# EPFL-IMOS/simple-SFOD

Measured on AMD Instinct MI355X. Metric: teacher+student train images/s on 1024x2048 synthetic, higher is better.
Workload: dtype bf16x3

## Files before the change

include/sfod_hip.h:

```cpp
#ifndef SFOD_HIP_H
#define SFOD_HIP_H
#include <stdint.h>
#ifdef __cplusplus
extern "C" {
#endif

#define SFOD_F32 0
#define SFOD_BF16 1
#define SFOD_BF16X3 2
#define SFOD_F16X3 3

int sfod_version(void);
const char* sfod_last_error(void);

int sfod_preprocess(const void* const* img_ptrs, const int32_t* sizes, int B, int Hp, int Wp,
                    int Cpad, const float* mean3, const float* std3, void* out, int dt,
                    void* stream);

int sfod_hflip_u8(const void* src, void* dst, int C, int H, int W, void* stream);

int sfod_resize_bilinear_u8(const void* src, void* dst, int C, int H, int W, int h, int w,
                            const int32_t* hbounds, const int32_t* hcoef, int ksize_h,
                            const int32_t* vbounds, const int32_t* vcoef, int ksize_v, int flip,
                            void* stream);
int sfod_resize_bilinear_u8_opt(const void* src, void* dst, int C, int H, int W, int y0, int x0, int ch, int cw,
                                int h, int w, const int32_t* hbounds, const int32_t* hcoef, int ksize_h,
                                const int32_t* vbounds, const int32_t* vcoef, int ksize_v, int flip_mode,
                                void* stream);

int sfod_conv_fwd(const void* x, const void* w, const float* bias, void* y, int B, int H, int W,
                  int Cin, int Cout, int ksize, int ldy, int act, float* stats, int dt, int out_dt,
                  void* stream);
int sfod_conv_fwd_ws(const void* x, const void* w, const uint32_t* w_absmax, const float* bias, void* y, int B, int H,
                     int W, int Cin, int Cout, int ksize, int ldy, int act, float* stats, int dt, int out_dt,
                     void* stream);
int64_t sfod_conv_fwd_scratch_bytes(int B, int H, int W, int Cin, int Cout, int ksize, int dt, int out_dt, int with_stats);
int sfod_conv_fwd_scratch(const void* x, const void* w, const uint32_t* w_absmax, const float* bias, void* y, int B, int H,
                          int W, int Cin, int Cout, int ksize, int ldy, int act, float* stats, int dt, int out_dt,
                          void* scratch, int64_t scratch_bytes, void* stream);
int sfod_conv_stats_blocks(int B, int H, int W, int Cin, int Cout, int ksize, int dt);
int sfod_set_conv_algo(int algo);
int sfod_conv_dgrad_bnred_blocks(int B, int H, int W, int Cin, int Cout, int dt);
int sfod_conv_dgrad_bnred(const void* x, const void* w, void* dz, int B, int H, int W, int Cin, int Cout, int dt,
                          const float* y, const float* mean, const float* invstd, const float* gamma,
                          const float* beta, float* red_ws, void* stream);
int sfod_conv_fwd_bnin_supported(int B, int H, int W, int Cin, int Cout, int dt);
int sfod_conv_fwd_bnin(const float* x_pre, const float* in_mean, const float* in_invstd, const float* in_gamma,
                       const float* in_beta, const void* w, const float* bias, float* y, int B, int H, int W, int Cin,
                       int Cout, int ldy, int act, float* stats, int dt, void* stream);
int sfod_set_gemm_tile(int tile);
int sfod_set_conv3x3_variant(int variant);
int sfod_last_conv_kernel(char* buf, int n);
int sfod_set_deterministic(int on);
int sfod_get_deterministic(void);
int sfod_set_conv3x3_m16(int on);
int sfod_set_wgrad3x3_pipe(int on);
int sfod_conv_fwd_algo(int B, int H, int W, int Cin, int Cout, int ksize, int dt);

int sfod_conv_first_supported(int B, int H, int W, int Cin, int Cout, int dt, int ldy);
int sfod_conv_first_fused(const void* x, const void* w, const float* bias, const float* scale,
                          const float* shift, void* y, float* stats, int B, int H, int W, int ldy,
                          int act, int dt, void* stream);
int sfod_conv_first_fused_ws(const void* x, const void* w, const uint32_t* w_absmax, const float* bias,
                             const float* scale, const float* shift, void* y, float* stats, int B, int H, int W,
                             int ldy, int act, int dt, void* stream);

int64_t sfod_conv_wgrad_ws_bytes(int B, int H, int W, int Cin, int Cout, int ksize, int lddy, int dt);
int sfod_conv_wgrad(const void* x, const void* dy, float* dw, int B, int H, int W, int Cin,
                    int Cout, int ksize, int lddy, int dt, void* ws, int64_t ws_bytes, void* stream);
int sfod_conv_wgrad_oihw_supported(int B, int H, int W, int Cin, int Cout, int ksize, int lddy, int dt);
int sfod_conv_wgrad_oihw(const void* x, const void* dy, float* dw_oihw, int B, int H, int W, int Cin,
                         int Cout, int ksize, int lddy, int dt, int accumulate, void* ws,
                         int64_t ws_bytes, void* stream);

int sfod_pack_conv_weight(const float* w_oihw, void* w_packed, int Cout, int Cin, int ksize,
                          int CinPad, int rot180, int dt, void* stream);
int sfod_pack_conv_weight_ws(const float* w_oihw, void* w_packed, uint32_t* absmax, int Cout, int Cin, int ksize,
                             int CinPad, int rot180, int dt, void* stream);
int sfod_pack_conv_weights_blocks(int Cout, int Cin, int ksize, int innerPad, int rot180);
int sfod_pack_conv_weights_multi(const int64_t* desc, int n, int total_blocks, int dt, void* stream);
int sfod_pack_conv_weights_multi_ws(const int64_t* desc, int n, int total_blocks, int dt, uint32_t* absmax ,
                                    void* stream);
int sfod_unpack_conv_wgrad(const float* dw_packed, float* dw_oihw, int Cout, int Cin, int ksize,
                           int CinPad, int accumulate, void* stream);
int sfod_pack_fc_weight(const float* w, void* out, int N, int K, int chw_c, int transpose, int dt,
                        void* stream);
int sfod_unpack_fc_wgrad(const float* dw_packed, float* dw, int N, int K, int chw_c,
                         int accumulate, void* stream);
int sfod_pack_fc_weight_ld(const float* w, void* out, int N, int K, int chw_c, int transpose, int ld,
                           int dt, void* stream);
int sfod_pack_fc_weight_ld_ws(const float* w, void* out, uint32_t* absmax, int N, int K, int chw_c, int transpose,
                              int ld, int dt, void* stream);
int sfod_unpack_fc_wgrad_ld(const float* dw_packed, float* dw, int N, int K, int chw_c, int ld,
                            int accumulate, void* stream);
int sfod_bias_grad(const void* dy, float* db, int M, int N, int ld, int accumulate, int dt,
                   void* stream);

int sfod_bn_finalize(const float* stats, int nblocks, int M, int C,
                     float* mean, float* invstd, float* running_mean, float* running_var,
                     float momentum, float eps, int update_running, int64_t* num_batches_tracked,
                     float* ws, void* stream);
int sfod_set_bn_finalize_fused(int on);
int sfod_bn_finalize_ws_floats(int C);
int sfod_bn_relu_pool_fwd(const void* y, const float* mean, const float* invstd,
                          const float* gamma, const float* beta, void* z, int B, int H, int W,
                          int C, int pool, int dt, int out_dt, void* stream);
int sfod_bn_relu_pool_fwd2(const void* y, const float* mean, const float* invstd,
                           const float* gamma, const float* beta, void* z, void* z2, int B, int H, int W,
                           int C, int pool, int dt, int out_dt, void* stream);
int sfod_bn_add_relu_fwd(const void* y, const float* mean, const float* invstd, const float* gamma,
                         const float* beta, const void* residual, void* z, void* z_pairs, void* z_pairs2, int64_t rows,
                         int C, int dt, int pairs_dt, void* stream);
int sfod_bn_relu_pool_bwd(const void* dz, const void* y, const float* mean, const float* invstd,
                          const float* gamma, const float* beta, void* dy, float* dgamma,
                          float* dbeta, float* dgamma_acc, float* dbeta_acc, float* ws, int B, int H,
                          int W, int C, int pool, int dt, int out_dt, int reduced_blocks, void* stream);
#define SFOD_BN_BWD_SCRATCH_ROWS 32
int sfod_bn_bwd_ws_floats(int M, int C);
int sfod_add_act(const void* a, const void* b, void* out, void* out_pairs, void* out_pairs2, int64_t n, int act, int dt,
                 int pairs_dt, void* stream);
int sfod_subsample2(const void* src, void* dst, int B, int H, int W, int C, int backward, int dt,
                    void* stream);
int sfod_stem7x7_supported(int B, int H, int W, int Cp, int dt);
int sfod_stem7x7(const float* x, const void* w_packed, const uint32_t* w_absmax, const float* bias, float* y, int B, int H,
                 int W, int Cp, int act, int dt, void* stream);
int sfod_im2col_stem(const void* x, void* out, int B, int H, int W, int Cp, int Kpad, int dt, int out_dt,
                     void* stream);
int sfod_maxpool3s2(const void* x, void* y, int B, int H, int W, int C, int dt, void* stream);
int sfod_act_bwd(void* dy, const void* y, int64_t n, int act, int dt, void* stream);
int sfod_add_inplace(void* a, const void* b, int64_t n, int dt, void* stream);
int sfod_add_act_bwd(void* a, const void* b, const void* y, int64_t n, int dt, void* stream);
int sfod_mul_mask(void* a, const uint8_t* mask, int64_t n, float scale, int dt, void* stream);

int sfod_rpn_decode(const float* rpn_out, int ld, const float* cell_anchors, int A, int B, int Hf,
                    int Wf, int stride, const int32_t* image_sizes, float* props, float* scores,
                    int32_t* flags, void* stream);
int sfod_rpn_decode_opt(const float* rpn_out, int ld, const float* cell_anchors, int A, int B, int Hf,
                        int Wf, int stride, const int32_t* image_sizes, float* props, float* scores,
                        int32_t* flags, float wx, float wy, float ww, float wh, void* stream);
int64_t sfod_sort_ws_bytes(int B, int n);
int sfod_segmented_sort_desc(const float* keys, int B, int n, float* out_keys, int32_t* out_idx,
                             void* ws, int64_t ws_bytes, void* stream);
int sfod_rpn_gather_topk(const float* props, const float* sorted_scores, const int32_t* sorted_idx,
                         int B, int NA, int k, float* cand_boxes, float* cand_scores,
                         uint8_t* cand_valid, void* stream);
// ... 125 lines not shown
```

simple-sfod_amd/csrc/elementwise.hip:

```cpp
#include "conv_internal.h"
#include <type_traits>
#include <atomic>
#include <stdlib.h>

template <typename T> struct VecT;
template <> struct VecT<float> {
  static constexpr int N = 4;
  typedef float4 raw;
};
template <> struct VecT<bf16_t> {
  static constexpr int N = 8;
  typedef uint4 raw;
};

template <> struct VecT<split_t> {
  static constexpr int N = 8;
  typedef uint4 raw;
};
template <> struct VecT<splith_t> {
  static constexpr int N = 8;
  typedef uint4 raw;
};

template <typename T> __device__ __forceinline__ void load_vec(const T* p, float* out);
// ... 1676 lines not shown
                                 int transpose, int ld, const unsigned* __restrict__ amax) {
  const float ws = amax != nullptr ? wscale_from_absmax(*amax) : 1.0f;
  const int rows = transpose ? K : N;
  const int64_t total = (int64_t)rows * ld;
  const int PP = chw_c > 0 ? K / chw_c : 1;
  for (int64_t t = (int64_t)blockIdx.x * blockDim.x + threadIdx.x; t < total;
       t += (int64_t)gridDim.x * blockDim.x) {
    const int inner = (int)(t % ld);
    const int row = (int)(t / ld);
    const int n = transpose ? inner : row;
    const int kp = transpose ? row : inner;
    float v = 0.f;
    if (n < N && kp < K) {
      int k = kp;
      if (chw_c > 0) { const int p = kp / chw_c, c = kp % chw_c; k = c * PP + p; }
      v = w[(int64_t)n * K + k];
    }
    put_elem<T>(out, t, v * ws);
  }
}

template <typename T>
__global__ void __launch_bounds__(256)
k_pack_fc_chw(const float* __restrict__ w, T* __restrict__ out, int N, int C, int PP, int ld,
              const unsigned* __restrict__ amax) {
  const float ws = amax != nullptr ? wscale_from_absmax(*amax) : 1.0f;
  extern __shared__ float tile[];
  const int n = blockIdx.y, c0 = blockIdx.x * 64;
  const int cw = min(64, C - c0);
  const float* src = w + (int64_t)n * C * PP + (int64_t)c0 * PP;
  for (int i = threadIdx.x; i < cw * PP; i += 256) tile[i] = src[i];
  __syncthreads();
  T* dst = out + (int64_t)n * ld;
  for (int j = threadIdx.x; j < PP * 64; j += 256) {
    const int p = j >> 6, cl = j & 63;
    if (cl < cw) put_elem<T>(dst, (int64_t)p * C + c0 + cl, tile[cl * PP + p] * ws);
  }
}

template <typename T>
__global__ void __launch_bounds__(256)
k_pack_fc_chw_t(const float* __restrict__ w, T* __restrict__ out, int N, int C, int PP, int ld,
                const unsigned* __restrict__ amax) {
  const float ws = amax != nullptr ? wscale_from_absmax(*amax) : 1.0f;
  extern __shared__ float tile[];
  const int n0 = blockIdx.y * 64, c0 = blockIdx.x * 4;
  const int nw = min(64, N - n0), cw = min(4, C - c0);
  const int run = cw * PP, pitch = 4 * PP + 1;
  for (int i = threadIdx.x; i < nw * run; i += 256) {
    const int nl = i / run, r = i - nl * run;
    tile[nl * pitch + r] = w[(int64_t)(n0 + nl) * C * PP + (int64_t)c0 * PP + r];
  }
  __syncthreads();
  for (int j = threadIdx.x; j < run * 64; j += 256) {
    const int r = j >> 6, nl = j & 63;
    if (nl < nw) {
      const int cl = r / PP, p = r - cl * PP;
      put_elem<T>(out, ((int64_t)p * C + c0 + cl) * ld + n0 + nl, tile[nl * pitch + r] * ws);
    }
  }
}

extern "C" int sfod_pack_fc_weight_ld_ws(const float* w, void* out, uint32_t* absmax, int N, int K, int chw_c,
                                         int transpose, int ld, int dt, void* stream) {
  SFOD_REQUIRE_EXTENTS("pack_fc_weight_ld_ws", N, K, chw_c, ld);
  SFOD_REQUIRE(ld >= (transpose ? N : K), "pack_fc_weight: ld too small");
  SFOD_REQUIRE(!sfod_is_pairs(dt) || ld % 8 == 0, "pack_fc_weight: operand pairs need ld % 8 == 0");
  SFOD_REQUIRE(absmax == nullptr || dt == SFOD_F16X3, "pack_fc_weight: the per-tensor scale belongs to SFOD_F16X3");
  hipStream_t s = (hipStream_t)stream;
  if (absmax != nullptr) {
    const int rc = launch_weight_absmax(w, (int64_t)N * K, nullptr, 1, absmax, s);
    if (rc) return rc;
  }
  const unsigned* am = absmax;
  const unsigned* none = nullptr;
  if (chw_c > 0 && K % chw_c == 0 && K / chw_c <= 64 && (int64_t)N * K >= (1 << 20) &&
      ld == (transpose ? N : K)) {
    const int C = chw_c, PP = K / chw_c;
    if (!transpose) {
      const dim3 grid(cdiv(C, 64), N);
      const size_t lds = (size_t)64 * PP * 4;
      if (dt == SFOD_F32) hipLaunchKernelGGL(k_pack_fc_chw<float>, grid, dim3(256), lds, s, w, (float*)out, N, C, PP, ld, none);
      else if (dt == SFOD_BF16X3) hipLaunchKernelGGL(k_pack_fc_chw<split_t>, grid, dim3(256), lds, s, w, (split_t*)out, N, C, PP, ld, none);
      else if (dt == SFOD_F16X3) hipLaunchKernelGGL(k_pack_fc_chw<splith_t>, grid, dim3(256), lds, s, w, (splith_t*)out, N, C, PP, ld, am);
      else hipLaunchKernelGGL(k_pack_fc_chw<bf16_t>, grid, dim3(256), lds, s, w, (bf16_t*)out, N, C, PP, ld, none);
    } else {
      const dim3 grid(cdiv(C, 4), cdiv(N, 64));
      const size_t lds = (size_t)64 * (4 * PP + 1) * 4;
      if (dt == SFOD_F32) hipLaunchKernelGGL(k_pack_fc_chw_t<float>, grid, dim3(256), lds, s, w, (float*)out, N, C, PP, ld, none);
      else if (dt == SFOD_BF16X3) hipLaunchKernelGGL(k_pack_fc_chw_t<split_t>, grid, dim3(256), lds, s, w, (split_t*)out, N, C, PP, ld, none);
      else if (dt == SFOD_F16X3) hipLaunchKernelGGL(k_pack_fc_chw_t<splith_t>, grid, dim3(256), lds, s, w, (splith_t*)out, N, C, PP, ld, am);
      else hipLaunchKernelGGL(k_pack_fc_chw_t<bf16_t>, grid, dim3(256), lds, s, w, (bf16_t*)out, N, C, PP, ld, none);
    }
    return sfod_check_launch("pack_fc_weight(chw)");
  }
  const int64_t total = (int64_t)(transpose ? K : N) * ld;
  if (dt == SFOD_BF16X3)
    hipLaunchKernelGGL(k_pack_fc_weight<split_t>, dim3(ew_grid(total)), dim3(256), 0, s, w, (split_t*)out, N, K, chw_c, transpose, ld, none);
  else if (dt == SFOD_F16X3)
    hipLaunchKernelGGL(k_pack_fc_weight<splith_t>, dim3(ew_grid(total)), dim3(256), 0, s, w, (splith_t*)out, N, K, chw_c, transpose, ld, am);
  else if (dt == SFOD_F32)
    hipLaunchKernelGGL(k_pack_fc_weight<float>, dim3(ew_grid(total)), dim3(256), 0, s, w, (float*)out, N, K, chw_c, transpose, ld, none);
  else
    hipLaunchKernelGGL(k_pack_fc_weight<bf16_t>, dim3(ew_grid(total)), dim3(256), 0, s, w, (bf16_t*)out, N, K, chw_c, transpose, ld, none);
  return sfod_check_launch("pack_fc_weight");
}

extern "C" int sfod_pack_fc_weight_ld(const float* w, void* out, int N, int K, int chw_c, int transpose,
                                      int ld, int dt, void* stream) {
  SFOD_REQUIRE_EXTENTS("pack_fc_weight_ld", N, K, chw_c, ld);
  return sfod_pack_fc_weight_ld_ws(w, out, nullptr, N, K, chw_c, transpose, ld, dt, stream);
}

extern "C" int sfod_pack_fc_weight(const float* w, void* out, int N, int K, int chw_c, int transpose,
                                   int dt, void* stream) {
  SFOD_REQUIRE_EXTENTS("pack_fc_weight", N, K, chw_c);
  return sfod_pack_fc_weight_ld(w, out, N, K, chw_c, transpose, transpose ? N : K, dt, stream);
}

__global__ void k_unpack_fc_wgrad(const float* __restrict__ dwp, float* __restrict__ dw, int N, int K,
                                  int chw_c, int ld, int accumulate) {
  const int64_t total = (int64_t)N * K;
  const int PP = chw_c > 0 ? K / chw_c : 1;
  for (int64_t t = (int64_t)blockIdx.x * blockDim.x + threadIdx.x; t < total;
       t += (int64_t)gridDim.x * blockDim.x) {
    const int k = (int)(t % K);
    const int n = (int)(t / K);
    int kp = k;
    if (chw_c > 0) { const int c = k / PP, p = k % PP; kp = p * chw_c + c; }
    const float v = dwp[(int64_t)n * ld + kp];
    dw[t] = accumulate ? dw[t] + v : v;
  }
}

__global__ void __launch_bounds__(256)
k_unpack_fc_chw(const float* __restrict__ dwp, float* __restrict__ dw, int C, int PP, int ld, int accumulate) {
  extern __shared__ float tile[];
  const int n = blockIdx.y, c0 = blockIdx.x * 64;
  const int cw = min(64, C - c0);
  const float* src = dwp + (int64_t)n * ld;
  for (int j = threadIdx.x; j < PP * 64; j += 256) {
    const int p = j >> 6, cl = j & 63;
    if (cl < cw) tile[cl * PP + p] = src[(int64_t)p * C + c0 + cl];
  }
  __syncthreads();
// ... 510 lines not shown
```

simple-sfod_amd/csrc/gemm_conv.hip:

```cpp
#include "conv_internal.h"
#include <algorithm>
#include <atomic>

typedef __attribute__((ext_vector_type(8))) __bf16 bf16x8;
typedef __attribute__((ext_vector_type(4))) short s16x4;
typedef __attribute__((ext_vector_type(8))) short s16x8;
typedef __attribute__((ext_vector_type(16))) float f32x16;
typedef __attribute__((ext_vector_type(4))) float f32x4;

#define LDS_PTR(p) ((__attribute__((address_space(3))) void*)(p))
#define GLB_PTR(p) ((const __attribute__((address_space(1))) void*)(p))

__device__ __attribute__((aligned(16))) unsigned int g_zero_page[64];

struct ConvArgs {
  int M;
  int H, W;
  int Cin;
  int Cout;
  int ks;
  int cpt_shift;
  int kchunks;
  int ldy;
  int act;
// ... 1257 lines not shown
        acc.x += v.x; acc.y += v.y; acc.z += v.z; acc.w += v.w;
      }
      *reinterpret_cast<float4*>(dw + i) = acc;
    } else {
      for (int64_t e = i; e < n && e < i + 4; ++e) {
        float acc = dw[e];
        for (int sl = 0; sl < nslab; ++sl) acc += ws[sl * stride + e];
        dw[e] = acc;
      }
    }
  }
}

struct GenWgradPlan { int wide, tiles_n, tiles_m, splits, pps; };
static GenWgradPlan gen_wgrad_plan(int M, int Cout, int Ntot, int dt) {
  GenWgradPlan g;
  const int split = (dt == SFOD_BF16X3);
  g.wide = split && Cout >= 128 && Ntot >= 256 && g_conv_algo != 3 &&
           (g_conv_algo == 4 || (int64_t)((Ntot + 255) / 256) * ((Cout + 127) / 128) >= 256);
  if (g.wide) {
    constexpr int BKP = 32;
    g.tiles_n = (Ntot + 255) / 256; g.tiles_m = (Cout + 127) / 128;
    const int tiles = g.tiles_n * g.tiles_m;
    const int max_splits = std::max(1, M / (8 * BKP));
    int best = 1;
    double best_eff = 0.0;
    for (int sp = 1; sp <= std::min(max_splits, 512); ++sp) {
      const int64_t wgs = (int64_t)tiles * sp;
      const double eff = (double)wgs / (double)((wgs + 255) / 256 * 256);
      if (eff > best_eff + 1e-9) { best_eff = eff; best = sp; }
      if (eff >= 0.85 && wgs >= 512) { best = sp; break; }
      if (wgs >= 4096) break;
    }
    int pps = (M + best - 1) / best;
    pps = (pps + BKP - 1) / BKP * BKP;
    g.pps = pps;
    g.splits = (M + pps - 1) / pps;
    return g;
  }
  const int BKP = (dt == SFOD_F32) ? 32 : 64;
  const int TILE = split ? 64 : 128;
  g.tiles_n = (Ntot + TILE - 1) / TILE; g.tiles_m = (Cout + TILE - 1) / TILE;
  int splits = (1024 + g.tiles_n * g.tiles_m - 1) / (g.tiles_n * g.tiles_m);
  const int max_splits = (M + BKP - 1) / BKP;
  if (splits > max_splits) splits = max_splits;
  if (splits < 1) splits = 1;
  int pps = (M + splits - 1) / splits;
  pps = (pps + BKP - 1) / BKP * BKP;
  g.pps = pps;
  g.splits = (M + pps - 1) / pps;
  return g;
}

extern "C" int64_t sfod_conv_wgrad_ws_bytes(int B, int H, int W, int Cin, int Cout, int ksize, int lddy, int dt) {
  if (!(conv_shape_fits(B, H, W, Cin, Cout, ksize) && sfod_ints_ok({lddy}))) return 0;
  int nb = 0;
  if (dt != SFOD_F32) {
    const W3Plan p = w3_plan_chunked(B, H, W, Cin, Cout, ksize, lddy, dt, nb);
    if (nb > 0) return p.ws_bytes;
  }
  if (!sfod_deterministic() || (int64_t)B * H * W == 0) return 0;
  const int Ntot = ksize * ksize * Cin;
  const GenWgradPlan g = gen_wgrad_plan(B * H * W, Cout, Ntot, dt);
  return g.splits > 1 ? (int64_t)g.splits * Cout * Ntot * 4 : 0;
}

extern "C" int sfod_conv_wgrad_oihw_supported(int B, int H, int W, int Cin, int Cout, int ksize, int lddy, int dt) {
  if (!(conv_shape_fits(B, H, W, Cin, Cout, ksize) && sfod_ints_ok({lddy}))) return 0;
  int nb;
  w3_plan_chunked(B, H, W, Cin, Cout, ksize, lddy, dt, nb);
  return nb > 0 ? 1 : 0;
}

extern "C" int sfod_conv_wgrad_oihw(const void* x, const void* dy, float* dw_oihw, int B, int H, int W, int Cin,
                                    int Cout, int ksize, int lddy, int dt, int accumulate, void* ws,
                                    int64_t ws_bytes, void* stream) {
  sfod_note_conv_kernel(nullptr);
  SFOD_REQUIRE(conv_shape_fits(B, H, W, Cin, Cout, ksize) && sfod_ints_ok({lddy}) && sfod_i64s_ok({ws_bytes}),
               "conv_wgrad_oihw: negative or oversized extent");
  SFOD_REQUIRE(x != nullptr && dy != nullptr && dw_oihw != nullptr, "conv_wgrad_oihw: null operand");
  SFOD_REQUIRE(lddy >= Cout, "conv_wgrad_oihw: lddy < Cout");
  int nb;
  w3_plan_chunked(B, H, W, Cin, Cout, ksize, lddy, dt, nb);
  SFOD_REQUIRE(nb > 0, "wgrad_oihw: shape not served by the halo-patch kernel (query sfod_conv_wgrad_oihw_supported)");
  return w3_launch_chunked(x, dy, dw_oihw, ws, ws_bytes, B, H, W, Cin, Cout, lddy, dt, accumulate ? 2 : 1, nb,
                           (hipStream_t)stream);
}

extern "C" int sfod_conv_wgrad(const void* x, const void* dy, float* dw, int B, int H, int W, int Cin,
                               int Cout, int ksize, int lddy, int dt, void* ws, int64_t ws_bytes,
                               void* stream) {
  sfod_note_conv_kernel(nullptr);
  SFOD_REQUIRE(conv_shape_fits(B, H, W, Cin, Cout, ksize) && sfod_ints_ok({lddy}) && sfod_i64s_ok({ws_bytes}),
               "conv_wgrad: negative or oversized extent");
  SFOD_REQUIRE(x != nullptr && dy != nullptr && dw != nullptr, "conv_wgrad: null operand");
  SFOD_REQUIRE(lddy >= Cout, "conv_wgrad: lddy < Cout");
  SFOD_REQUIRE(ksize == 1 || ksize == 3, "wgrad: ksize must be 1 or 3");
  SFOD_REQUIRE(dt == SFOD_F32 || dt == SFOD_BF16 || dt == SFOD_BF16X3, "wgrad: unknown dt");
  const int E = (dt == SFOD_F32) ? 4 : 8;
  SFOD_REQUIRE(Cin % E == 0 && lddy % E == 0, "wgrad: Cin / lddy must be multiples of the 16-byte chunk (bf16x3: of 8)");
  if ((int64_t)B * H * W == 0) return 0;
  const int split = (dt == SFOD_BF16X3);
  SFOD_REQUIRE(!split || Cout % 8 == 0, "wgrad: bf16x3 needs Cout % 8 == 0");
  {
    int nb;
    w3_plan_chunked(B, H, W, Cin, Cout, ksize, lddy, dt, nb);
    if (nb > 0) return w3_launch_chunked(x, dy, dw, ws, ws_bytes, B, H, W, Cin, Cout, lddy, dt, 0, nb, (hipStream_t)stream);
  }
  hipStream_t s = (hipStream_t)stream;
  float* dw_out = dw;
  WgradArgs a;
  a.M = B * H * W; a.H = H; a.W = W; a.Cin = Cin; a.Cout = Cout; a.ks = ksize; a.lddy = lddy;
  const int cpt = Cin / E;
  a.cpt_shift = 0;
  if (ksize == 3) {
    a.cpt_shift = ilog2_exact(cpt);
    SFOD_REQUIRE(a.cpt_shift >= 0, "wgrad3x3: Cin/chunk must be a power of two");
  }
  a.nchunks = ksize * ksize * cpt;
  a.Ntot = ksize * ksize * Cin;
  if (a.M == 0) return 0;
  const GenWgradPlan g = gen_wgrad_plan(a.M, Cout, a.Ntot, dt);
  a.pix_per_split = g.pps;
  a.tiles_n = g.tiles_n;
  a.tiles_m = g.tiles_m;
  a.slab_stride = 0;
  const bool slabs = sfod_deterministic() && g.splits > 1;
  if (slabs) {
    const int64_t need = (int64_t)g.splits * Cout * a.Ntot * 4;
    if (ws == nullptr || ws_bytes < need) {
      sfod_set_error("wgrad: deterministic mode needs the workspace of sfod_conv_wgrad_ws_bytes");
      return SFOD_EBADARG;
    }
    a.slab_stride = (int64_t)Cout * a.Ntot;
    dw_out = (float*)ws;
  }
  const int tiles = g.tiles_n * g.tiles_m;
  if (g.wide) {
    constexpr int LDS = 3 * 32 * (128 + 256) * 4;
    static const hipError_t attr_rc = hipFuncSetAttribute(reinterpret_cast<const void*>(k_conv_wgrad_x3w),
                                                          hipFuncAttributeMaxDynamicSharedMemorySize, LDS);
    SFOD_REQUIRE(attr_rc == hipSuccess, "wgrad: cannot raise the dynamic LDS limit");
    sfod_note_conv_kernel("k_conv_wgrad_x3w");
    hipLaunchKernelGGL(k_conv_wgrad_x3w, dim3(tiles * g.splits), dim3(512), LDS, s, (const bf16_t*)x, (const bf16_t*)dy,
                       dw_out, a);
  } else {
    dim3 grid(tiles * g.splits);
    sfod_note_conv_kernel(dt == SFOD_F32 ? "k_conv_wgrad<float,2,2,0>"
                                         : (split ? "k_conv_wgrad<bf16_t,2,2,1>" : "k_conv_wgrad<bf16_t,2,2,0>"));
    if (dt == SFOD_F32)
      hipLaunchKernelGGL((k_conv_wgrad<float, 2, 2>), grid, dim3(256), 2 * 2 * 32 * 512, s, (const float*)x,
                         (const float*)dy, dw_out, a);
    else if (split)
      hipLaunchKernelGGL((k_conv_wgrad<bf16_t, 2, 2, true>), grid, dim3(256), 2 * 2 * 64 * 256, s, (const bf16_t*)x,
                         (const bf16_t*)dy, dw_out, a);
    else
      hipLaunchKernelGGL((k_conv_wgrad<bf16_t, 2, 2>), grid, dim3(256), 2 * 2 * 64 * 256, s, (const bf16_t*)x,
                         (const bf16_t*)dy, dw_out, a);
  }
  int rc = sfod_check_launch(g.wide ? "conv_wgrad_x3w" : "conv_wgrad");
  if (rc == 0 && slabs) {
    const int64_t n = (int64_t)Cout * a.Ntot;
// ... 7 lines not shown
```

simple-sfod_amd/modeling/roi_heads.py:

```python
import math

import torch
import torch.nn as nn

from .. import native
from ..registry import ROI_BOX_HEAD_REGISTRY, ROI_HEADS_REGISTRY
from ..structures import Boxes, Instances, ShapeSpec
from .offchain import OffChain as _OffChain, heads_on as _heads_on
from .batched import BatchedDetections, BatchedGT, BatchedProposals
from .box_regression import ROI_DEFAULT_WEIGHTS, roi_box_reg_options
from .roi_pooler import roi_pooler_options


class ROIPooler(nn.Module):

    def __init__(self, output_size, scales, sampling_ratio, pooler_type, prefix="MODEL.ROI_BOX_HEAD"):
        super().__init__()
        assert len(scales) == 1
        output_size, self.sampling_ratio, self.aligned = roi_pooler_options(output_size, sampling_ratio, pooler_type, prefix)
        self.pooler_type = pooler_type
        self.options = {} if (self.sampling_ratio == 0 and self.aligned) else \
            {"sampling_ratio": self.sampling_ratio, "aligned": self.aligned}
        self.output_size = (output_size, output_size)
        self.scale = scales[0]
# ... 248 lines not shown
        pk = self.__dict__.pop("_packed", None) or {}
        pooled = native.roi_align_fwd(feat, rois, self.pooled, self.box_pooler.scale, **self.box_pooler.options)
        R = pooled.shape[0]
        x0 = pooled.view(R, PP * C)
        w1 = pk["w1"] if pk else native.pack_fc_weight(bh.fc1.weight.detach(), dt, chw_c=C)
        h1 = native.conv_fwd(x0, w1, bh.fc1.bias.detach(), bh.fc1.out_features, 1, act=1)
        w2 = pk["w2"] if pk else native.pack_fc_weight(bh.fc2.weight.detach(), dt)
        h2 = native.conv_fwd(h1, w2, bh.fc2.bias.detach(), bh.fc2.out_features, 1, act=1)
        wp = pk["wp"] if pk else torch.cat([bp.cls_score.weight.detach(), bp.bbox_pred.weight.detach()])
        bpb = pk["bpb"] if pk else torch.cat([bp.cls_score.bias.detach(), bp.bbox_pred.bias.detach()])
        wpp = pk["wpp"] if pk else native.pack_fc_weight(wp, dt)
        pred = native.conv_fwd(h2, wpp, bpb, wp.shape[0], 1, out_dtype=torch.float32, ldy=self.pred_ld)
        st = {"x0": x0, "h1": h1, "h2": h2, "pred": pred, "wp": wp, "feat_shape": tuple(feat.shape)}
        for k in ("wpt", "w2t", "w1t"):
            if k in pk:
                st[k] = pk[k]
        return st

    def _box_backward(self, st, rois, d_pred, feat_shape_nchw):
        dtype = native.grad_dtype_of(self.compute_dtype)
        dt = native.dt_of_dtype(dtype)
        bh = self.box_head
        K = self.num_classes
        NP = self.pred_cols
        d_pred_c = native.cast(d_pred, dtype)
        off = _OffChain(_heads_on(d_pred))
        dwp, dbp = off.run(lambda: (native.conv_wgrad(st["h2"], d_pred_c, NP, 1, operand=dtype).view(NP, -1),
                                    native.bias_grad(d_pred, NP)), st["h2"], d_pred_c, d_pred)
        wpt = st.get("wpt")
        if wpt is None:
            wpt = native.pack_fc_weight(st["wp"], dt, transpose=True, ld=self.pred_ld)
        dh2 = native.conv_fwd(d_pred_c, wpt, None, bh.fc2.out_features, 1)
        dfeat, (dw1, db1, dw2, db2) = self._box_head_backward(st, rois, dh2)
        off.join(dwp, dbp)
        pgrads = [dw1, db1, dw2, db2, dwp[: K + 1].contiguous(), dbp[: K + 1].contiguous(),
                  dwp[K + 1:].contiguous(), dbp[K + 1:].contiguous()]
        return dfeat, pgrads

    def _box_head_backward(self, st, rois, dh2):
        dtype = native.grad_dtype_of(self.compute_dtype)
        dt = native.dt_of_dtype(dtype)
        bh = self.box_head
        C = self.channels
        native.act_bwd_(dh2, st["h2"], 1)
        off = _OffChain(_heads_on(dh2))
        dw2, db2 = off.run(lambda: (native.conv_wgrad(st["h1"], dh2, bh.fc2.out_features, 1, operand=dtype).view(bh.fc2.out_features, -1),
                                    native.bias_grad(dh2, bh.fc2.out_features)), st["h1"], dh2)
        w2t = st.get("w2t")
        if w2t is None:
            w2t = native.pack_fc_weight(bh.fc2.weight.detach(), dt, transpose=True)
        dh1 = native.conv_fwd(dh2, w2t, None, bh.fc2.in_features, 1)
        native.act_bwd_(dh1, st["h1"], 1)
        def fc1_param_grads():
            dw1p = native.conv_wgrad(st["x0"], dh1, bh.fc1.out_features, 1, operand=dtype).view(bh.fc1.out_features, -1)
            dw1_ = native.grad_sink(bh.fc1.weight)
            if dw1_ is not None:
                native.unpack_fc_wgrad(dw1p, dw1_, chw_c=C, accumulate=True)
                dw1_ = None
            else:
                dw1_ = torch.empty_like(bh.fc1.weight)
                native.unpack_fc_wgrad(dw1p, dw1_, chw_c=C)
            return dw1_, native.bias_grad(dh1, bh.fc1.out_features)

        dw1, db1 = off.run(fc1_param_grads, st["x0"], dh1)
        w1t = st.get("w1t")
        if w1t is None:
            w1t = native.pack_fc_weight(bh.fc1.weight.detach(), dt, chw_c=C, transpose=True)
        dx0 = native.conv_fwd(dh1, w1t, None, bh.fc1.in_features, 1)
        B, H, W, _ = st["feat_shape"]
        dfeat = native.roi_align_bwd(dx0.view(-1, self.pooled * self.pooled, C), rois, (B, H, W, C), self.pooled,
                                     self.box_pooler.scale, **self.box_pooler.options)
        off.join(dw1, db1, dw2, db2)
        return dfeat.permute(0, 3, 1, 2), [dw1, db1, dw2, db2]

    @torch.no_grad()
    def label_and_sample_proposals(self, proposals, targets, branch="", keys=None):
        props = proposals
        B, P, _ = props.boxes.shape
        if self.proposal_append_gt:
            boxes, count = native.append_gt(props.boxes, props.count, targets.boxes, targets.count)
        else:
            boxes, count = props.boxes, props.count
        matched, cls = native.roi_match(boxes, count, targets.boxes, targets.classes, targets.count,
                                        self.iou_threshold, self.num_classes)
        keys = keys if keys is not None else getattr(self, "_forced_keys", None)
        if keys is None:
            keys = torch.randint(0, 2 ** 31 - 1, (B, boxes.shape[1]), dtype=torch.int32, device=boxes.device)
        sidx, scnt = native.subsample_roi(cls, keys, self.batch_size_per_image, self.positive_fraction,
                                          self.num_classes)
        rois, gt_cls, gt_box, n_valid = native.roi_build_samples(boxes, cls, matched, sidx, scnt, targets.boxes,
                                                                 targets.count)
        return {"rois": rois, "gt_cls": gt_cls, "gt_box": gt_box, "n_valid": n_valid, "count": scnt,
                "sampled_idxs": sidx, "image_sizes": props.image_sizes}

    @torch.no_grad()
    def _inference(self, feat, proposals, sizes_dev=None):
        rois = native.make_rois(proposals.boxes, proposals.count)
        st = self._box_forward(feat, rois)
        bp = self.box_predictor
        if sizes_dev is None:
            sizes_dev = native.dev_const(tuple((int(s[0]), int(s[1])) for s in proposals.image_sizes), torch.int32,
                                         feat.device)
        out = native.frcnn_inference(st["pred"], self.num_classes, proposals.boxes, proposals.count, sizes_dev,
                                     bp.test_score_thresh, bp.test_nms_thresh, bp.test_topk_per_image,
                                     self.bbox_threshold, self.nms_numel_limit, box_reg=bp._box_reg)
        return BatchedDetections(out, proposals.image_sizes), st["pred"]
# ... 60 lines not shown
```

simple-sfod_amd/native.py:

```python
import collections
import ctypes
import os
import re
import warnings

import torch

warnings.filterwarnings("ignore", message="ComplexHalf support is experimental")

_HERE = os.path.dirname(os.path.abspath(__file__))
HEADER = os.path.join(os.path.dirname(_HERE), "include", "sfod_hip.h")
SO_PATH = os.environ.get("SFOD_HIP_LIB", os.path.join(_HERE, "lib", "libsfod_hip.so"))

F32, BF16, BF16X3, F16X3 = 0, 1, 2, 3

SPLIT_DTYPE = torch.complex32
SPLITH_DTYPE = torch.uint32
PAIR_DTYPES = (SPLIT_DTYPE, SPLITH_DTYPE)

COMPUTE_MODES = {"fp32": F32, "bf16": BF16, "bf16x3": BF16X3, "f16x3": F16X3}


def mode_dt(name):
    try:
# ... 155 lines not shown
    return as_operand(t, dtype), as_operand(t, gdt)


class _Everything:
    def __contains__(self, item):
        return True


class KernelTimer:

    def __init__(self, watch=("sfod_conv_fwd", "sfod_conv_wgrad", "sfod_conv_wgrad_oihw")):
        self.watch = _Everything() if watch is None else set(watch)
        self.records = []

    def summary(self):
        torch.cuda.synchronize()
        out = {}
        for name, flops, a, b in self.records:
            d = out.setdefault(name, {"launches": 0, "ms": 0.0, "flops": 0.0})
            d["launches"] += 1
            d["ms"] += a.elapsed_time(b)
            d["flops"] += flops
        return out


_timer = None


def set_timer(timer):
    global _timer
    _timer = timer


def call(name, *args, timer_name=None, flops=0.0, tag=""):
    lib = load()
    conv = [(_p(a) if isinstance(a, torch.Tensor) else a) for a in args]
    if _timer is not None and (timer_name or name) in _timer.watch:
        a, b = torch.cuda.Event(enable_timing=True), torch.cuda.Event(enable_timing=True)
        a.record()
        rc = getattr(lib, name)(*conv, _stream())
        b.record()
        _timer.records.append(((timer_name or name) + tag, flops, a, b))
    else:
        rc = getattr(lib, name)(*conv, _stream())
    _chk(rc, name)


def query(name, *args):
    return getattr(load(), name)(*args)


def set_conv_algo(algo):
    load().sfod_set_conv_algo(int(algo))


def set_wgrad3x3_pipe(on):
    load().sfod_set_wgrad3x3_pipe(int(on))


def set_gemm_tile(tile):
    load().sfod_set_gemm_tile(int(tile))


def set_conv3x3_variant(variant):
    load().sfod_set_conv3x3_variant(int(variant))


def last_conv_kernel():
    buf = ctypes.create_string_buffer(256)
    n = load().sfod_last_conv_kernel(buf, len(buf))
    if n < 0:
        _chk(n, "sfod_last_conv_kernel")
    return buf.value.decode()


def set_deterministic(on):
    lib = load()
    prev = bool(lib.sfod_get_deterministic())
    lib.sfod_set_deterministic(int(bool(on)))
    return prev


def set_bn_finalize_fused(on):
    load().sfod_set_bn_finalize_fused(int(bool(on)))


def set_conv3x3_m16(on):
    load().sfod_set_conv3x3_m16(int(on))


_const_cache = {}


def dev_const(values, dtype, device):
    key = (values, dtype, str(device))
    t = _const_cache.get(key)
    if t is None:
        if len(_const_cache) > 4096:
            _const_cache.clear()
        t = torch.tensor(values, dtype=dtype).to(device)
        _const_cache[key] = t
    return t


_PIN_SLOTS, _PIN_WIDTH = 32, 64
_pin_ring = {}
# ... 379 lines not shown
    if x.dim() != 4 or x.dtype not in (torch.bfloat16,) + PAIR_DTYPES:
        return False
    B, H, W, cin = x.shape
    return bool(query("sfod_conv_first_supported", B, H, W, cin, cout, dt_of(x), cout))


def conv_first_stats(x, w_packed, bias):
    B, H, W, cin = x.shape
    stats = _stats_buffer(B, H, W, cin, 64, 3, dt_of(x), x.device)
    call("sfod_conv_first_fused_ws", x, w_packed, wscale_of(w_packed), bias, None, None, None, stats, B, H, W, 64, 0,
         dt_of(x))
    return stats


def conv_first_apply(x, w_packed, bias, scale, shift, relu=True):
    B, H, W, cin = x.shape
    z = torch.empty(B, H, W, 64, dtype=x.dtype, device=x.device)
    call("sfod_conv_first_fused_ws", x, w_packed, wscale_of(w_packed), bias, scale, shift, z, None, B, H, W, 64,
         1 if relu else 0, dt_of(x))
    return z


_ws_cache = {}


def _workspace(dev, nbytes):
    key = (dev, _stream())
    cur = _ws_cache.get(key)
    if cur is None or cur.numel() < nbytes:
        cur = torch.empty(int(nbytes), dtype=torch.uint8, device=dev)
        _ws_cache[key] = cur
    return cur


def conv_wgrad(x, dy, cout, ksize, dw_packed=None, operand=None):
    operand = operand or x.dtype
    x, dy = as_operand(x, operand), as_operand(dy, operand)
    dt = dt_of(x)
    if x.dim() == 2:
        B, H, W, cin = x.shape[0], 1, 1, x.shape[1]
    else:
        B, H, W, cin = x.shape
    lddy = dy.shape[-1]
    cout_k = (cout + 7) // 8 * 8 if dt in (BF16X3, F16X3) else cout
    assert cout_k <= lddy, "dy narrower than the padded output-channel count"
    if dw_packed is None or cout_k != cout:
        assert dw_packed is None, "accumulating bf16x3 weight gradients needs Cout % 8 == 0"
        dw_packed = torch.zeros(cout_k, ksize * ksize, cin, dtype=torch.float32, device=x.device)
    nbytes = query("sfod_conv_wgrad_ws_bytes", B, H, W, cin, cout_k, ksize, lddy, dt)
    ws = _workspace(x.device, nbytes) if nbytes > 0 else None
    call("sfod_conv_wgrad", x, dy, dw_packed, B, H, W, cin, cout_k, ksize, lddy, dt, ws, nbytes,
         flops=2.0 * B * H * W * cout * ksize * ksize * cin)
    return dw_packed if cout_k == cout else dw_packed[:cout]


def conv_wgrad_oihw_supported(x, dy, cout, ksize):
    if x.dim() != 4:
        return False
    B, H, W, cin = x.shape
    if dt_of(x) == BF16X3 and (cout % 8 or dy.shape[-1] % 8):
        return False
    return bool(query("sfod_conv_wgrad_oihw_supported", B, H, W, cin, cout, ksize, dy.shape[-1], dt_of(x)))


def conv_wgrad_oihw(x, dy, dw_oihw, accumulate=False):
    cout, cin, ksize, _ = dw_oihw.shape
    B, H, W, cinp = x.shape
    assert cinp == cin and dw_oihw.is_contiguous() and dw_oihw.dtype == torch.float32
    dy = as_operand(dy, x.dtype)
    lddy = dy.shape[-1]
    dt = dt_of(x)
    nbytes = query("sfod_conv_wgrad_ws_bytes", B, H, W, cin, cout, ksize, lddy, dt)
    ws = _workspace(x.device, nbytes)
    call("sfod_conv_wgrad_oihw", x, dy, dw_oihw, B, H, W, cin, cout, ksize, lddy, dt, int(accumulate), ws, nbytes,
         flops=2.0 * B * H * W * cout * ksize * ksize * cin)
    return dw_oihw


def conv_weight_grad(x, dy, weight, operand=None):
    operand = operand or x.dtype
    x, dy = as_operand(x, operand), as_operand(dy, operand)
    cout, cin, k, _ = weight.shape
    sink = grad_sink(weight)
    if sink is not None and k == 3 and x.shape[-1] == cin and conv_wgrad_oihw_supported(x, dy, cout, 3):
        conv_wgrad_oihw(x, dy, sink, accumulate=True)
        return None
    if sink is not None and k == 1 and x.shape[-1] == cin and (dt_of(x) != BF16X3 or cout % 8 == 0):
        conv_wgrad(x, dy, cout, 1, dw_packed=sink.view(cout, 1, cin))
        return None
    dwp = conv_wgrad(x, dy, cout, k)
    if sink is not None:
        unpack_conv_wgrad(dwp, sink, accumulate=True)
        return None
    dw = torch.empty_like(weight)
    unpack_conv_wgrad(dwp, dw)
    return dw


def bias_grad(dy, n, db=None, accumulate=False):
    m = dy.numel() // dy.shape[-1]
    if db is None:
        db = torch.empty(n, dtype=torch.float32, device=dy.device)
    call("sfod_bias_grad", dy, db, m, n, dy.shape[-1], int(accumulate), dt_of(dy))
    return db


# ... 485 lines not shown
```

Baseline: 161.2.

## Route large FC weight gradients through transposed-pair GEMM with split-K slabs

Adds a weight-gradient path for large 1x1/FC layers in bf16x3. Both x and dy are transposed into row-padded pair layouts, then the existing tiled conv GEMM kernel runs with the row dimension as K, split into several slabs chosen by a small cost model. The slabs are then summed, and the result is unpacked straight into the OIHW or CHW weight gradient. The ROI box-head fc1 backward uses this path, and the generic conv_wgrad also uses it when workspace is available. It also vectorizes the transposed CHW FC weight pack store when N%8==0. It costs extra workspace and transpose passes, and the path is gated by heuristic shape thresholds.

```diff
diff --git a/include/sfod_hip.h b/include/sfod_hip.h
--- a/include/sfod_hip.h
+++ b/include/sfod_hip.h
@@ -40,6 +40,11 @@
                           void* scratch, int64_t scratch_bytes, void* stream);
 int sfod_conv_stats_blocks(int B, int H, int W, int Cin, int Cout, int ksize, int dt);
 int sfod_set_conv_algo(int algo);
+int sfod_set_fc_wgrad_splits(int splits);
+int sfod_fc_wgrad_direct_supported(int R, int Cin, int Cout, int lddy, int dt);
+int sfod_fc_wgrad_direct(const void* x, const void* dy, float* dw, int R, int Cin, int Cout, int lddy, int chw_c,
+                         int accumulate, int dt, void* ws, int64_t ws_bytes, void* stream);
+int sfod_pairs_transpose(const void* in, void* out, int R, int N, int ldi, int Rpad, void* stream);
 int sfod_conv_dgrad_bnred_blocks(int B, int H, int W, int Cin, int Cout, int dt);
 int sfod_conv_dgrad_bnred(const void* x, const void* w, void* dz, int B, int H, int W, int Cin, int Cout, int dt,
                           const float* y, const float* mean, const float* invstd, const float* gamma,
@@ -91,6 +96,7 @@
                            int dt, void* stream);
 int sfod_pack_fc_weight_ld_ws(const float* w, void* out, uint32_t* absmax, int N, int K, int chw_c, int transpose,
                               int ld, int dt, void* stream);
+int sfod_pack_fc_chw_t(const float* w, void* out, uint32_t* absmax, int N, int C, int PP, int dt, void* stream);
 int sfod_unpack_fc_wgrad_ld(const float* dw_packed, float* dw, int N, int K, int chw_c, int ld,
                             int accumulate, void* stream);
 int sfod_bias_grad(const void* dy, float* db, int M, int N, int ld, int accumulate, int dt,
diff --git a/simple-sfod_amd/csrc/elementwise.hip b/simple-sfod_amd/csrc/elementwise.hip
--- a/simple-sfod_amd/csrc/elementwise.hip
+++ b/simple-sfod_amd/csrc/elementwise.hip
@@ -1752,6 +1752,20 @@
     tile[nl * pitch + r] = w[(int64_t)(n0 + nl) * C * PP + (int64_t)c0 * PP + r];
   }
   __syncthreads();
+  if (N % 8 == 0) {
+    for (int j = threadIdx.x; j < run * 8; j += 256) {
+      const int r = j >> 3, g = j & 7;
+      if (g * 8 >= nw) continue;
+      const int cl = r / PP, p = r - cl * PP;
+      float v[8];
+#pragma unroll
+      for (int i = 0; i < 8; ++i) v[i] = tile[(g * 8 + i) * pitch + r] * ws;
+      T* dst = out + ((int64_t)p * C + c0 + cl) * ld + n0 + g * 8;
+      store_vec<T>(dst, v);
+      if constexpr (sizeof(T) == 4 && VecT<T>::N == 4) store_vec<T>(dst + 4, v + 4);
+    }
+    return;
+  }
   for (int j = threadIdx.x; j < run * 64; j += 256) {
     const int r = j >> 6, nl = j & 63;
     if (nl < nw) {
@@ -1759,6 +1773,33 @@
       put_elem<T>(out, ((int64_t)p * C + c0 + cl) * ld + n0 + nl, tile[nl * pitch + r] * ws);
     }
   }
+}
+
+static void launch_pack_fc_chw_t(const float* w, void* out, const unsigned* am, int N, int C, int PP, int dt, hipStream_t s) {
+  const unsigned* none = nullptr;
+  const dim3 grid(cdiv(C, 4), cdiv(N, 64));
+  const size_t lds = (size_t)64 * (4 * PP + 1) * 4;
+  if (dt == SFOD_F32) hipLaunchKernelGGL(k_pack_fc_chw_t<float>, grid, dim3(256), lds, s, w, (float*)out, N, C, PP, N, none);
+  else if (dt == SFOD_BF16X3) hipLaunchKernelGGL(k_pack_fc_chw_t<split_t>, grid, dim3(256), lds, s, w, (split_t*)out, N, C, PP, N, none);
+  else if (dt == SFOD_F16X3) hipLaunchKernelGGL(k_pack_fc_chw_t<splith_t>, grid, dim3(256), lds, s, w, (splith_t*)out, N, C, PP, N, am);
+  else hipLaunchKernelGGL(k_pack_fc_chw_t<bf16_t>, grid, dim3(256), lds, s, w, (bf16_t*)out, N, C, PP, N, none);
+}
+
+extern "C" int sfod_pack_fc_chw_t(const float* w, void* out, uint32_t* absmax, int N, int C, int PP, int dt, void* stream) {
+  SFOD_REQUIRE_EXTENTS("pack_fc_chw_t", N, C, PP);
+  SFOD_REQUIRE(w != nullptr && out != nullptr, "pack_fc_chw_t: null operand");
+  SFOD_REQUIRE(dt == SFOD_F32 || dt == SFOD_BF16 || sfod_is_pairs(dt), "pack_fc_chw_t: unknown dt");
+  SFOD_REQUIRE(PP >= 1 && PP <= 63 && sfod_prod_fits({N, C, PP}, 1LL << 40), "pack_fc_chw_t: 1 <= PP <= 63, N * C * PP below 2^40");
+  SFOD_REQUIRE(!sfod_is_pairs(dt) || N % 8 == 0, "pack_fc_chw_t: operand pairs need N % 8 == 0");
+  SFOD_REQUIRE(absmax == nullptr || dt == SFOD_F16X3, "pack_fc_chw_t: the per-tensor scale belongs to SFOD_F16X3");
+  if (N == 0 || C == 0) return 0;
+  hipStream_t s = (hipStream_t)stream;
+  if (absmax != nullptr) {
+    const int rc = launch_weight_absmax(w, (int64_t)N * C * PP, nullptr, 1, absmax, s);
+    if (rc) return rc;
+  }
+  launch_pack_fc_chw_t(w, out, absmax, N, C, PP, dt, s);
+  return sfod_check_launch("pack_fc_chw_t");
 }
 
 extern "C" int sfod_pack_fc_weight_ld_ws(const float* w, void* out, uint32_t* absmax, int N, int K, int chw_c,
@@ -1785,12 +1826,7 @@
       else if (dt == SFOD_F16X3) hipLaunchKernelGGL(k_pack_fc_chw<splith_t>, grid, dim3(256), lds, s, w, (splith_t*)out, N, C, PP, ld, am);
       else hipLaunchKernelGGL(k_pack_fc_chw<bf16_t>, grid, dim3(256), lds, s, w, (bf16_t*)out, N, C, PP, ld, none);
     } else {
-      const dim3 grid(cdiv(C, 4), cdiv(N, 64));
-      const size_t lds = (size_t)64 * (4 * PP + 1) * 4;
-      if (dt == SFOD_F32) hipLaunchKernelGGL(k_pack_fc_chw_t<float>, grid, dim3(256), lds, s, w, (float*)out, N, C, PP, ld, none);
-      else if (dt == SFOD_BF16X3) hipLaunchKernelGGL(k_pack_fc_chw_t<split_t>, grid, dim3(256), lds, s, w, (split_t*)out, N, C, PP, ld, none);
-      else if (dt == SFOD_F16X3) hipLaunchKernelGGL(k_pack_fc_chw_t<splith_t>, grid, dim3(256), lds, s, w, (splith_t*)out, N, C, PP, ld, am);
-      else hipLaunchKernelGGL(k_pack_fc_chw_t<bf16_t>, grid, dim3(256), lds, s, w, (bf16_t*)out, N, C, PP, ld, none);
+      launch_pack_fc_chw_t(w, out, am, N, C, PP, dt, s);
     }
     return sfod_check_launch("pack_fc_weight(chw)");
   }
diff --git a/simple-sfod_amd/csrc/gemm_conv.hip b/simple-sfod_amd/csrc/gemm_conv.hip
--- a/simple-sfod_amd/csrc/gemm_conv.hip
+++ b/simple-sfod_amd/csrc/gemm_conv.hip
@@ -1333,12 +1333,170 @@
   return g;
 }
 
+__global__ void __launch_bounds__(256)
+k_pairs_transpose(const uint4* __restrict__ in, uint4* __restrict__ out, int R, int N, int ldi, int Rpad) {
+  __shared__ __attribute__((aligned(16))) unsigned char tl[2 * 64 * 128];
+  const int n0 = blockIdx.x * 64, r0 = blockIdx.y * 64;
+#pragma unroll
+  for (int i = 0; i < 4; ++i) {
+    const int c = threadIdx.x + 256 * i;
+    const int rl = c >> 4, g = (c >> 1) & 7, part = c & 1;
+    const int r = r0 + rl, n = n0 + g * 8;
+    uint4 v = make_uint4(0u, 0u, 0u, 0u);
+    if (r < R && n < N) v = in[((int64_t)r * ldi + n) / 4 + part];
+    const uint32_t w[4] = {v.x, v.y, v.z, v.w};
+    unsigned char* base = tl + part * 8192 + (((rl >> 3) ^ g) << 4) + (rl & 7) * 2;
+#pragma unroll
+    for (int j = 0; j < 8; ++j)
+      *reinterpret_cast<unsigned short*>(base + (g * 8 + j) * 128) = (unsigned short)(w[j >> 1] >> (16 * (j & 1)));
+  }
+  __syncthreads();
+#pragma unroll
+  for (int i = 0; i < 4; ++i) {
+    const int c = threadIdx.x + 256 * i;
+    const int nl = c >> 4, rg = (c >> 1) & 7, part = c & 1;
+    const int n = n0 + nl, r = r0 + rg * 8;
+    if (n < N && r < Rpad)
+      out[((int64_t)n * Rpad + r) / 4 + part] =
+          *reinterpret_cast<const uint4*>(tl + part * 8192 + nl * 128 + ((rg ^ ((nl >> 3) & 7)) << 4));
+  }
+}
+
+extern "C" int sfod_pairs_transpose(const void* in, void* out, int R, int N, int ldi, int Rpad, void* stream) {
+  SFOD_REQUIRE_EXTENTS("pairs_transpose", R, N, ldi, Rpad);
+  SFOD_REQUIRE(in != nullptr && out != nullptr, "pairs_transpose: null operand");
+  SFOD_REQUIRE(N % 8 == 0 && ldi % 8 == 0 && Rpad % 8 == 0 && ldi >= N && Rpad >= R, "pairs_transpose: N, ldi, Rpad in whole 8-groups");
+  SFOD_REQUIRE(Rpad <= (1 << 22), "pairs_transpose: too many rows");
+  if (N == 0 || Rpad == 0) return 0;
+  hipLaunchKernelGGL(k_pairs_transpose, dim3(cdiv(N, 64), cdiv(Rpad, 64)), dim3(256), 0, (hipStream_t)stream,
+                     (const uint4*)in, (uint4*)out, R, N, ldi, Rpad);
+  return sfod_check_launch("pairs_transpose");
+}
+
+static std::atomic<int> g_fc_wgrad_splits{0};
+extern "C" int sfod_set_fc_wgrad_splits(int s) {
+  g_fc_wgrad_splits.store((s >= 0 && s <= 16) ? s : 0, std::memory_order_relaxed);
+  return 0;
+}
+
+struct FcWgradPlan { int use, Rpad, S; int64_t xt_bytes, dyt_bytes, slab_elems, total; };
+static FcWgradPlan fc_wgrad_plan(int M, int Cin, int Cout, int ksize, int dt) {
+  FcWgradPlan p{};
+  static const int on = []() { const char* e = getenv("SFOD_FC_WGRAD_GEMM"); return e ? atoi(e) : 1; }();
+  const int algo = g_conv_algo;
+  if (ksize != 1 || dt != SFOD_BF16X3 || M < 1 || M > (1 << 20) || Cin % 8 != 0 || Cout % 8 != 0) return p;
+  if (algo != 5) {
+    if (!on || algo == 3 || algo == 4) return p;
+    if (M < 512 || M > 8192 || (int64_t)Cin * Cout < (1 << 24)) return p;
+  }
+  p.Rpad = (M + 15) / 16 * 16;
+  if (!sfod_prod_fits({Cin, p.Rpad, 4}, 1LL << 38) || !sfod_prod_fits({Cout, p.Rpad, 4}, 1LL << 38) ||
+      !sfod_prod_fits({Cout, Cin, 4 * 16}, 1LL << 38))
+    return p;
+  const int KT = p.Rpad / 16;
+  const int64_t tiles = (int64_t)((Cout + 255) / 256) * ((Cin + 255) / 256);
+  int S = g_fc_wgrad_splits.load(std::memory_order_relaxed);
+  if (S <= 0) {
+    double best = 1e300;
+    S = 1;
+    for (int s = 1; s <= 16 && (s == 1 || KT / s >= 8); ++s) {
+      const double rounds = (double)((tiles * s + 255) / 256);
+      const double t = rounds * (((KT + s - 1) / s) * 1.3 + 6.0) + (2 * s + 2) * (double)Cout * Cin * 4.0 / 3.5e6;
+      if (t < best * 0.97) { best = t; S = s; }
+    }
+  }
+  if (S > KT) S = KT;
+  p.S = S;
+  p.xt_bytes = (int64_t)Cin * p.Rpad * 4;
+  p.dyt_bytes = (int64_t)Cout * p.Rpad * 4;
+  p.slab_elems = (int64_t)Cout * Cin;
+  p.total = p.xt_bytes + p.dyt_bytes + (int64_t)S * p.slab_elems * 4;
+  p.use = p.total <= (1LL << 40);
+  return p;
+}
+
+static int fc_wgrad_gemm(const FcWgradPlan& p, const void* x, const void* dy, int M, int Cin, int Cout, int lddy, void* ws,
+                         int& nslab, hipStream_t s) {
+  uint4* xt = (uint4*)ws;
+  uint4* dyt = (uint4*)((char*)ws + p.xt_bytes);
+  float* slabs = (float*)((char*)ws + p.xt_bytes + p.dyt_bytes);
+  hipLaunchKernelGGL(k_pairs_transpose, dim3(cdiv(Cin, 64), cdiv(p.Rpad, 64)), dim3(256), 0, s, (const uint4*)x, xt, M, Cin,
+                     Cin, p.Rpad);
+  hipLaunchKernelGGL(k_pairs_transpose, dim3(cdiv(Cout, 64), cdiv(p.Rpad, 64)), dim3(256), 0, s, (const uint4*)dy, dyt, M,
+                     Cout, lddy, p.Rpad);
+  int rc = sfod_check_launch("pairs_transpose");
+  if (rc) return rc;
+  ConvArgs a;
+  a.wamax = nullptr;
+  a.M = Cout; a.H = 1; a.W = 1; a.Cin = 2 * p.Rpad; a.Cout = Cin; a.ks = 1; a.cpt_shift = 0;
+  a.kchunks = 2 * p.Rpad / 8;
+  a.ldy = Cin; a.act = 0;
+  a.kt_per = 0; a.nsplit = 1; a.slab = p.slab_elems;
+  if (p.S > 1) {
+    const int KT = p.Rpad / 16;
+    a.kt_per = (KT + p.S - 1) / p.S;
+    a.nsplit = (KT + a.kt_per - 1) / a.kt_per;
+  }
+  rc = launch_one<bf16_t, float, 4, true, 4, 3, 1, 64>(dyt, xt, nullptr, slabs, nullptr, a, s);
+  if (rc) return rc;
+  sfod_note_conv_kernel("k_conv_wgrad_gemm<256,256>");
+  nslab = a.nsplit;
+  return 0;
+}
+
+static int fc_wgrad_slab_sum(const float* slabs, float* dst, int64_t n, int nslab, hipStream_t s) {
+  sfod_note_conv_kernel_then("k_wgrad_slab_sum");
+  hipLaunchKernelGGL(k_wgrad_slab_sum, dim3(cdiv(n, 1024) > 4096 ? 4096 : cdiv(n, 1024)), dim3(256), 0, s, slabs, dst, n,
+                     nslab, n);
+  return sfod_check_launch("wgrad_slab_sum");
+}
+
+static int fc_wgrad_launch(const FcWgradPlan& p, const void* x, const void* dy, float* dw, int M, int Cin, int Cout, int lddy,
+                           void* ws, hipStream_t s) {
+  int nslab = 1;
+  const int rc = fc_wgrad_gemm(p, x, dy, M, Cin, Cout, lddy, ws, nslab, s);
+  if (rc) return rc;
+  return fc_wgrad_slab_sum((const float*)((char*)ws + p.xt_bytes + p.dyt_bytes), dw, p.slab_elems, nslab, s);
+}
+
+extern "C" int sfod_fc_wgrad_direct_supported(int R, int Cin, int Cout, int lddy, int dt) {
+  if (!(conv_shape_fits(R, 1, 1, Cin, Cout, 1) && sfod_ints_ok({lddy})) || lddy < Cout || lddy % 8 != 0) return 0;
+  return fc_wgrad_plan(R, Cin, Cout, 1, dt).use ? 1 : 0;
+}
+
+extern "C" int sfod_fc_wgrad_direct(const void* x, const void* dy, float* dw, int R, int Cin, int Cout, int lddy, int chw_c,
+                                    int accumulate, int dt, void* ws, int64_t ws_bytes, void* stream) {
+  sfod_note_conv_kernel(nullptr);
+  SFOD_REQUIRE(conv_shape_fits(R, 1, 1, Cin, Cout, 1) && sfod_ints_ok({lddy, chw_c}) && sfod_i64s_ok({ws_bytes}),
+               "fc_wgrad_direct: negative or oversized extent");
+  SFOD_REQUIRE(x != nullptr && dy != nullptr && dw != nullptr, "fc_wgrad_direct: null operand");
+  SFOD_REQUIRE(lddy >= Cout && lddy % 8 == 0, "fc_wgrad_direct: lddy >= Cout, in whole 8-groups");
+  SFOD_REQUIRE(chw_c == 0 || Cin % chw_c == 0, "fc_wgrad_direct: Cin must be a multiple of chw_c");
+  const FcWgradPlan p = fc_wgrad_plan(R, Cin, Cout, 1, dt);
+  SFOD_REQUIRE(p.use, "fc_wgrad_direct: shape not served (query sfod_fc_wgrad_direct_supported)");
+  SFOD_REQUIRE(ws != nullptr && ws_bytes >= p.total, "fc_wgrad_direct: workspace too small (sfod_conv_wgrad_ws_bytes)");
+  hipStream_t s = (hipStream_t)stream;
+  int nslab = 1;
+  int rc = fc_wgrad_gemm(p, x, dy, R, Cin, Cout, lddy, ws, nslab, s);
+  if (rc) return rc;
+  float* slabs = (float*)((char*)ws + p.xt_bytes + p.dyt_bytes);
+  if (nslab > 1) {
+    rc = fc_wgrad_slab_sum(slabs + p.slab_elems, slabs, p.slab_elems, nslab - 1, s);
+    if (rc) return rc;
+  }
+  return sfod_unpack_fc_wgrad_ld(slabs, dw, Cout, Cin, chw_c, Cin, accumulate, stream);
+}
+
 extern "C" int64_t sfod_conv_wgrad_ws_bytes(int B, int H, int W, int Cin, int Cout, int ksize, int lddy, int dt) {
   if (!(conv_shape_fits(B, H, W, Cin, Cout, ksize) && sfod_ints_ok({lddy}))) return 0;
   int nb = 0;
   if (dt != SFOD_F32) {
     const W3Plan p = w3_plan_chunked(B, H, W, Cin, Cout, ksize, lddy, dt, nb);
     if (nb > 0) return p.ws_bytes;
+  }
+  if ((int64_t)B * H * W != 0) {
+    const FcWgradPlan f = fc_wgrad_plan(B * H * W, Cin, Cout, ksize, dt);
+    if (f.use) return f.total;
   }
   if (!sfod_deterministic() || (int64_t)B * H * W == 0) return 0;
   const int Ntot = ksize * ksize * Cin;
@@ -1389,6 +1547,13 @@
     if (nb > 0) return w3_launch_chunked(x, dy, dw, ws, ws_bytes, B, H, W, Cin, Cout, lddy, dt, 0, nb, (hipStream_t)stream);
   }
   hipStream_t s = (hipStream_t)stream;
+  {
+    const FcWgradPlan f = fc_wgrad_plan(B * H * W, Cin, Cout, ksize, dt);
+    if (f.use) {
+      if (ws != nullptr && ws_bytes >= f.total) return fc_wgrad_launch(f, x, dy, dw, B * H * W, Cin, Cout, lddy, ws, s);
+      SFOD_REQUIRE(g_conv_algo != 5, "wgrad: the GEMM form needs the workspace of sfod_conv_wgrad_ws_bytes");
+    }
+  }
   float* dw_out = dw;
   WgradArgs a;
   a.M = B * H * W; a.H = H; a.W = W; a.Cin = Cin; a.Cout = Cout; a.ks = ksize; a.lddy = lddy;
diff --git a/simple-sfod_amd/modeling/roi_heads.py b/simple-sfod_amd/modeling/roi_heads.py
--- a/simple-sfod_amd/modeling/roi_heads.py
+++ b/simple-sfod_amd/modeling/roi_heads.py
@@ -324,6 +324,11 @@
         dh1 = native.conv_fwd(dh2, w2t, None, bh.fc2.in_features, 1)
         native.act_bwd_(dh1, st["h1"], 1)
         def fc1_param_grads():
+            if native.fc_wgrad_direct_supported(st["x0"], bh.fc1.out_features, dh1.shape[-1], operand=dtype):
+                sink = native.grad_sink(bh.fc1.weight)
+                dw1_ = sink if sink is not None else torch.empty_like(bh.fc1.weight)
+                native.fc_wgrad_direct(st["x0"], dh1, dw1_, chw_c=C, accumulate=sink is not None, operand=dtype)
+                return (None if sink is not None else dw1_), native.bias_grad(dh1, bh.fc1.out_features)
             dw1p = native.conv_wgrad(st["x0"], dh1, bh.fc1.out_features, 1, operand=dtype).view(bh.fc1.out_features, -1)
             dw1_ = native.grad_sink(bh.fc1.weight)
             if dw1_ is not None:
diff --git a/simple-sfod_amd/native.py b/simple-sfod_amd/native.py
--- a/simple-sfod_amd/native.py
+++ b/simple-sfod_amd/native.py
@@ -231,6 +231,22 @@
 
 def set_conv_algo(algo):
     load().sfod_set_conv_algo(int(algo))
+
+
+def set_fc_wgrad_splits(splits):
+    load().sfod_set_fc_wgrad_splits(int(splits))
+
+
+def pairs_transpose(x, n=None, rpad=None, out=None):
+    assert x.dim() == 2 and x.dtype == SPLIT_DTYPE and x.is_contiguous()
+    R, ld = x.shape
+    n = ld if n is None else n
+    rpad = (R + 15) // 16 * 16 if rpad is None else rpad
+    if out is None:
+        out = torch.empty(n, rpad, dtype=SPLIT_DTYPE, device=x.device)
+    assert out.shape == (n, rpad) and out.dtype == SPLIT_DTYPE and out.is_contiguous()
+    call("sfod_pairs_transpose", x, out, R, n, ld, rpad)
+    return out
 
 
 def set_wgrad3x3_pipe(on):
@@ -716,6 +732,27 @@
     call("sfod_conv_wgrad", x, dy, dw_packed, B, H, W, cin, cout_k, ksize, lddy, dt, ws, nbytes,
          flops=2.0 * B * H * W * cout * ksize * ksize * cin)
     return dw_packed if cout_k == cout else dw_packed[:cout]
+
+
+def fc_wgrad_direct_supported(x, cout, lddy=None, operand=None):
+    operand = operand or x.dtype
+    lddy = cout if lddy is None else lddy
+    if x.dim() != 2 or operand != SPLIT_DTYPE or cout % 8 or lddy % 8:
+        return False
+    return bool(query("sfod_fc_wgrad_direct_supported", x.shape[0], x.shape[1], cout, lddy, BF16X3))
+
+
+def fc_wgrad_direct(x, dy, dw, chw_c=0, accumulate=False, operand=None):
+    operand = operand or x.dtype
+    x, dy = as_operand(x, operand), as_operand(dy, operand)
+    cout, cin = dw.shape
+    assert dw.is_contiguous() and dw.dtype == torch.float32 and x.shape[1] == cin
+    R, lddy, dt = x.shape[0], dy.shape[-1], dt_of(x)
+    nbytes = query("sfod_conv_wgrad_ws_bytes", R, 1, 1, cin, cout, 1, lddy, dt)
+    ws = _workspace(x.device, nbytes) if nbytes > 0 else None
+    call("sfod_fc_wgrad_direct", x, dy, dw, R, cin, cout, lddy, chw_c, int(accumulate), dt, ws, nbytes,
+         timer_name="sfod_conv_wgrad", flops=2.0 * R * cout * cin)
+    return dw
 
 
 def conv_wgrad_oihw_supported(x, dy, cout, ksize):
```

After: 161.5 (median of 6 runs). About the same (+0.1%).
